# Farama-Foundation/Metaworld

Measured on NVIDIA H100. Metric: env steps/sec MT50 batched (4096 envs/GPU) at 1/2/4/8 H100 vs CPU MuJoCo, higher is better.
Workload: dtype f32

## Files before the change

### include/metaworld_b200.h

```cpp
#ifndef METAWORLD_B200_H
#define METAWORLD_B200_H
#ifdef __cplusplus
extern "C" {
#endif

typedef struct mw_engine mw_engine;

enum mw_status { MW_OK = 0, MW_ERR_CUDA = -1, MW_ERR_ARG = -2, MW_ERR_STATE = -3 };

int mw_sizeof_model(void);
int mw_sizeof_taskconst(void);
int mw_sizeof_envstate(void);
int mw_sizeof_snapshot(void);
const char* mw_last_error(void);
const char* mw_build_info(void);

int mw_create(mw_engine** out, int device, int n_models, const void* models, const void* taskconsts,
              const float* const* meshverts, const int* nmeshvert);
void mw_destroy(mw_engine*);

int mw_set_envs(mw_engine*, int n_envs, const int* env_model);

int mw_build_snapshots(mw_engine*, int n, const int* model_idx, const double* rand_vec ,
                       const double* rand_vec_pass1 , const unsigned char* partially_observable,
// ... 21 lines not shown
int mw_set_options(mw_engine*, int max_episode_steps, int terminate_on_success, unsigned long long seed);
int mw_set_goal_sets(mw_engine*, const int* first , const int* count );

int mw_get_state(mw_engine*, void* out_host);
int mw_set_state(mw_engine*, const void* in_host);
int mw_debug_substeps(mw_engine*, int nstep, const float* ctrl2 , void* stream);
int mw_debug_forward(mw_engine*, const float* ctrl2 , float* dump, void* stream);
int mw_debug_dump_floats(void);
int mw_get_counters(mw_engine*, unsigned long long* out5);

int mw_rebalance(mw_engine*);

int mw_set_profiling(mw_engine*, int on);
int mw_get_env_profile(mw_engine*, unsigned* out );

int mw_get_profile(mw_engine*, unsigned long long* out13);
int mw_get_env_cost(mw_engine*, unsigned* out);

#ifdef __cplusplus
}
#endif
#endif
```

### metaworld_b200/csrc/mw_collide.cuh

```cuda
#pragma once
#include "mw_math.cuh"

#ifndef MW_WARP
#define MW_WARP 32
#endif

enum { G_PLANE = 0, G_HFIELD, G_SPHERE, G_CAPSULE, G_ELLIPSOID, G_CYLINDER, G_BOX, G_MESH };

struct RawCon { creal dist, pos[3], normal[3]; };

struct DShape {
  int type; const creal* pos; const creal* mat; creal size[3]; const float4* vert; int nvert;
};

DEV int plane_sphere_raw(const creal* pn, const creal* pp, const creal* c, creal r, creal margin, RawCon* o) {
  creal t[3]; v3sub(t, c, pp);
  creal dist = v3dot(t, pn) - r;
  if (dist > margin) return 0;
  o->dist = dist; v3copy(o->normal, pn);
  v3addscl(o->pos, c, pn, -(r + (creal)0.5 * dist));
  return 1;
}
DEV int plane_capsule(const DShape& a, const DShape& b, creal margin, RawCon* o) {
  creal n[3], ax[3], c[3]; mat_col(n, a.mat, 2); mat_col(ax, b.mat, 2);
// ... 376 lines not shown
    l[2] = dl[2] >= 0 ? s.size[1] : -s.size[1];
  } else if (s.type == G_CAPSULE) {
    l[0] = l[1] = 0; l[2] = dl[2] >= 0 ? s.size[1] : -s.size[1];
  } else {
    l[0] = l[1] = l[2] = 0;
  }
  mat_mulvec(out, s.mat, l); v3add(out, out, s.pos);
}
DEV creal core_radius(const DShape& s) { return (s.type == G_SPHERE || s.type == G_CAPSULE) ? s.size[0] : (creal)0; }
DEV void support_pair(const DShape& A, const DShape& B, const creal* dir, SV* o, int lane) {
  creal nd[3] = {-dir[0], -dir[1], -dir[2]};
  support_shape(A, dir, o->a, lane);
  support_shape(B, nd, o->b, lane);
  v3sub(o->v, o->a, o->b);
}
DEV void closest_tri(const creal* a, const creal* b, const creal* c, creal* w) {
  creal ab[3], ac[3], ap[3]; v3sub(ab, b, a); v3sub(ac, c, a); v3scl(ap, a, -1);
  creal d1 = v3dot(ab, ap), d2 = v3dot(ac, ap);
  if (d1 <= 0 && d2 <= 0) { w[0] = 1; w[1] = w[2] = 0; return; }
  creal bp[3]; v3scl(bp, b, -1);
  creal d3 = v3dot(ab, bp), d4 = v3dot(ac, bp);
  if (d3 >= 0 && d4 <= d3) { w[1] = 1; w[0] = w[2] = 0; return; }
  creal vc = d1 * d4 - d3 * d2;
  if (vc <= 0 && d1 >= 0 && d3 <= 0) { creal v = d1 / (d1 - d3); w[0] = 1 - v; w[1] = v; w[2] = 0; return; }
  creal cp[3]; v3scl(cp, c, -1);
  creal d5 = v3dot(ab, cp), d6 = v3dot(ac, cp);
  if (d6 >= 0 && d5 <= d6) { w[2] = 1; w[0] = w[1] = 0; return; }
  creal vb = d5 * d2 - d1 * d6;
  if (vb <= 0 && d2 >= 0 && d6 <= 0) { creal x = d2 / (d2 - d6); w[0] = 1 - x; w[1] = 0; w[2] = x; return; }
  creal va = d3 * d6 - d5 * d4;
// ... 207 lines not shown
  } else {
    dist = gr;
    const creal z0 = fmax(-h1, cz - h2), z1 = fmin(h1, cz + h2), zm = (creal)0.5 * (z0 + z1);
    for (int q = 0; q < 3; q++) { n[q] = u[q]; P[q] = A.pos[q] + (r1 + (creal)0.5 * gr) * u[q] + zm * a1[q]; }
  }
  if (dist > margin) return 0;
  o->dist = dist; v3copy(o->normal, n); v3copy(o->pos, P);
  return 1;
}

#define GJK_FINISH() {  \
    creal w4_[3]; simplex_weights(s, n, w4_); v3zero(fwa); v3zero(fwb); \
    for (int i_ = 0; i_ < n && i_ < 3; i_++) { v3addscl(fwa, fwa, s[i_].a, w4_[i_]); v3addscl(fwb, fwb, s[i_].b, w4_[i_]); } \
    creal dv_[3]; v3sub(dv_, fwb, fwa); fdcore = v3norm(dv_); \
    if (fdcore > (creal)1e-10) { outcome = 1; st = ST_DONE; } else { st = ST_G1; k = 0; } }
__device__ __noinline__ int convex_pair(const DShape& A, const DShape& B, creal margin, RawCon* o, EpaSm* E, EpaWs* W, int lane, long long* prof = nullptr) {
  const creal dirs[6][3] = {{1, 0, 0}, {-1, 0, 0}, {0, 1, 0}, {0, -1, 0}, {0, 0, 1}, {0, 0, -1}};
  const creal ra = core_radius(A), rb = core_radius(B);
  enum { ST_GJK0 = 0, ST_GJK, ST_G1, ST_G2, ST_G3, ST_EPA, ST_DONE };
  SV* const s = (SV*)E->fd;
  int n = 0; creal v[3];
  int st = ST_GJK0, git = 0, k = 0, sg = 0;
  int outcome = 0;
  creal ab[3] = {0, 0, 0}, gd[3] = {0, 0, 0}, nn[3] = {0, 0, 0}, vv = 0;
  creal dirl[3] = {1, 0, 0}, fwa[3] = {0, 0, 0}, fwb[3] = {0, 0, 0}, fdcore = 0;
  v3sub(v, A.pos, B.pos);
  if (v3dot(v, v) < (creal)1e-24) { v[0] = 1; v[1] = v[2] = 0; }
  for (int guard = 0; guard < 128; guard++) {
    if (lane == 0) {
      bool query = false;
      while (!query && st != ST_DONE && st != ST_EPA) {
// ... 23 lines not shown
          } else if (n != 3 || sg >= 2) { outcome = 3; st = ST_DONE; }
          else { if (sg == 0) v3copy(dirl, nn); else v3scl(dirl, nn, -1); query = true; }
        }
      }
    }
    const int stb = __shfl_sync(FULLMASK, st, 0);
    if (stb == ST_DONE || stb == ST_EPA) break;
    creal dir[3] = {bcast(dirl[0], 0), bcast(dirl[1], 0), bcast(dirl[2], 0)};
    SV w; support_pair(A, B, dir, &w, lane);
    int need_cs = 0;
    if (lane == 0) {
      if (st == ST_GJK0) { s[0] = w; n = 1; v3copy(v, w.v); st = ST_GJK; git = 0; }
      else if (st == ST_GJK) {
        const creal vw = v3dot(v, w.v);
        if (vv - vw <= (creal)1e-12 * vv || vv - vw <= GJK_TOL * sqrt(vv)) GJK_FINISH()
        else if (vw > 0 && vw / sqrt(vv) - ra - rb > margin + (creal)1e-4) { outcome = 3; st = ST_DONE; }
        else {
          bool dup = false;
          for (int i = 0; i < n; i++) { creal t[3]; v3sub(t, s[i].v, w.v); if (v3dot(t, t) < (creal)1e-24) dup = true; }
          if (dup) GJK_FINISH()
          else { s[n++] = w; need_cs = 1; }
        }
      } else if (st == ST_G1) {
        creal dd[3]; v3sub(dd, w.v, s[0].v);
        if (v3dot(dd, dd) > (creal)1e-20) s[n++] = w;
        k++;
      } else if (st == ST_G2) {
        creal aw[3], cr[3]; v3sub(aw, w.v, s[0].v); v3cross(cr, ab, aw);
        if (v3dot(cr, cr) > (creal)1e-20) s[n++] = w;
        else { sg++; if (sg == 2) { sg = 0; k++; } }
      } else if (st == ST_G3) {
// ... 73 lines not shown
      nf += ne;
      __syncwarp();
    }
  }
  int result = 0;
  RawCon rc; rc.dist = 0; v3zero(rc.pos); v3zero(rc.normal);
  if (lane == 0) {
    creal wa[3] = {0, 0, 0}, wb[3] = {0, 0, 0};
    bool have = false;
    if (outcome == 1) {
      const creal dist = fdcore - ra - rb;
      if (dist <= margin + (creal)1e-4) {
        creal dvec[3]; v3sub(dvec, fwb, fwa);
        v3scl(rc.normal, dvec, 1 / fdcore); rc.dist = dist; have = true;
        v3copy(wa, fwa); v3copy(wb, fwb);
      }
    } else if (outcome == 2 && bestf >= 0) {
      const int i0 = E->fv[0][bestf], i1 = E->fv[1][bestf], i2 = E->fv[2][bestf];
      creal w3[3]; closest_tri(E->vv[i0], E->vv[i1], E->vv[i2], w3);
      const int ids[3] = {i0, i1, i2};
      for (int q = 0; q < 3; q++) for (int c = 0; c < 3; c++) { wa[c] += W->va[ids[q]][c] * w3[q]; wb[c] += W->vb[ids[q]][c] * w3[q]; }
      const creal dist = -E->fd[bestf] - ra - rb;
      if (dist <= margin) { rc.dist = dist; rc.normal[0] = W->fn[0][bestf]; rc.normal[1] = W->fn[1][bestf]; rc.normal[2] = W->fn[2][bestf]; have = true; }
    }
    if (have) {
      for (int q = 0; q < 3; q++) rc.pos[q] = (creal)0.5 * (wa[q] + rc.normal[q] * ra + wb[q] - rc.normal[q] * rb);
      refine_cyl_box(A, B, &rc);
      result = rc.dist <= margin ? 1 : 0;
    }
    if (prof) { prof[10] += eit; prof[11] += git; }
  }
  __syncwarp();
  result = __shfl_sync(FULLMASK, result, 0);
  o->dist = bcast(rc.dist, 0);
  for (int q = 0; q < 3; q++) { o->pos[q] = bcast(rc.pos[q], 0); o->normal[q] = bcast(rc.normal[q], 0); }
  return result;
}
```

### metaworld_b200/csrc/mw_engine.cu

```cuda
#include <cuda_runtime.h>
#include <stdint.h>
#include <stdio.h>
#include <stdlib.h>
#include <string.h>

#include <algorithm>
#include <string>
#include <utility>
#include <vector>

#include "../../include/metaworld_b200.h"
#include "mw_tasks.cuh"

#ifndef WARPS_PER_BLOCK
#define WARPS_PER_BLOCK 7
#endif
#define BLOCK_THREADS (WARPS_PER_BLOCK * 32)
#define MW_ENVPROF_W 20

static thread_local std::string g_err;
static int fail(int code, const std::string& msg) { g_err = msg; return code; }
#define CK(x) do { cudaError_t e_ = (x); if (e_ != cudaSuccess) return fail(MW_ERR_CUDA, std::string(#x ": ") + cudaGetErrorString(e_)); } while (0)

struct EngineDev {
  const unsigned char* models; int model_stride;
  const MwTaskConst* taskconsts;
  const float* const* meshverts;
  MwEnvState* state; MwSnapshot* snaps;
  const int* goal_first; const int* goal_count;
  int* diag;
  EpaWs* epa;
  WarpSpill* spill;
  int slot_by_sm;
  unsigned long long* prof;
  unsigned long long* model_cycles;
  unsigned* env_cost;
  unsigned* env_cycles;
  unsigned* env_prof;
  int n_envs, max_steps, terminate_on_success; unsigned long long seed;
  int autoreset_mode;
};

DEV unsigned mw_smid() { unsigned r; asm volatile("mov.u32 %0, %%smid;" : "=r"(r)); return r; }
DEV size_t scratch_slot(const EngineDev& e, int warp) { return (size_t)(e.slot_by_sm ? mw_smid() : blockIdx.x) * WARPS_PER_BLOCK + warp; }
__global__ void k_nsmid(unsigned* out) { unsigned r; asm volatile("mov.u32 %0, %%nsmid;" : "=r"(r)); *out = r; }

struct BlockShared {
  alignas(16) unsigned char model[(sizeof(MwModel) + 15) / 16 * 16];
  MwTaskConst tc;
  CtaShare cs;
  alignas(8) unsigned long long bar;
};
// ... 11 lines not shown
    asm volatile("fence.proxy.async.shared::cta;" ::: "memory");
  }
  __syncthreads();
  if (threadIdx.x == 0) {
    asm volatile("mbarrier.arrive.expect_tx.shared::cta.b64 _, [%0], %1;" ::"r"(smem_u32(&bs->bar)), "r"(bytes) : "memory");
    asm volatile("cp.async.bulk.shared::cluster.global.mbarrier::complete_tx::bytes [%0], [%1], %2, [%3];" ::"r"(smem_u32(bs->model)), "l"(src), "r"(bytes), "r"(smem_u32(&bs->bar)) : "memory");
  }
  for (int i = threadIdx.x; i < (int)(sizeof(MwTaskConst) / 4); i += blockDim.x) ((int*)&bs->tc)[i] = ((const int*)tc_src)[i];
  unsigned ok = 0;
  do {
    asm volatile("{ .reg .pred p; mbarrier.try_wait.parity.shared::cta.b64 p, [%1], %2; selp.u32 %0, 1, 0, p; }" : "=r"(ok) : "r"(smem_u32(&bs->bar)), "r"(0u) : "memory");
  } while (!ok);
  __syncthreads();
}

DEV void join_cta(BlockShared* bs, WarpShared* wsa, WarpScratch* w, int warp, int live_warps) {
  if (threadIdx.x == 0) { bs->cs.q_head = 0; bs->cs.nwarp = live_warps; bs->cs.peer_stride = (int)sizeof(WarpShared); bs->cs.peer0 = (unsigned char*)wsa; }
  if ((threadIdx.x & 31) == 0) { w->cta = &bs->cs; w->warp_in_cta = warp; w->ncand = 0; w->prof_on = 0; w->nblk1 = mw_tree_split((const MwModel*)bs->model); }
#ifdef MW_CHOL_ONE_CHAIN
  if ((threadIdx.x & 31) == 0) w->nblk1 = ((const MwModel*)bs->model)->nv;
#endif
  __syncwarp();
}
__device__ void eng_forward(const TaskCtx& c, int lane) { mw_forward(c.m, c.meshvert, c.w, lane); }
__device__ void eng_sim(const TaskCtx& c, int nstep, int lane) {
  for (int s = 0; s < nstep; s++) { mw_forward(c.m, c.meshvert, c.w, lane); mw_euler(c.m, c.w, lane); }
}

DEV void load_env(WarpShared* ws, const MwEnvState* src, int lane) {
  ((float4*)&ws->es)[lane] = ((const float4*)src)[lane];
  SYNCW();
  WarpScratch* w = &ws->w;
  if (lane < MW_MAXNQ) { w->qposd[lane] = ws->es.qpos[lane]; w->qpos[lane] = (real)w->qposd[lane]; }
// ... 48 lines not shown
       const int* __restrict__ block_live) {
  extern __shared__ __align__(16) unsigned char smem[];
  BlockShared* bs = (BlockShared*)smem;
  WarpShared* wsa = (WarpShared*)(smem + sizeof(BlockShared));
  const int blk = block_order[blockIdx.x];
  if (block_live && !block_live[blk]) return;
  const int mi = block_model[blk];
  stage_model(bs, e.models + (size_t)mi * e.model_stride, (unsigned)sizeof(bs->model), e.taskconsts + mi);
  const int warp = threadIdx.x >> 5, lane = threadIdx.x & 31;
  if (warp >= block_count[blk]) return;
  const int env = perm[block_start[blk] + warp];
  WarpShared* ws = wsa + warp;
  ws->w.epa = e.epa + scratch_slot(e, warp);
  ws->w.sp = e.spill + scratch_slot(e, warp);
  WarpScratch* w = &ws->w;
  join_cta(bs, wsa, w, warp, block_count[blk]);
  const MwModel* m = (const MwModel*)bs->model;
  load_env(ws, e.state + env, lane);
  const bool ended = DEFERRED && ws->es.ended != 0.f;
  if (lane < 16) w->prof[lane] = 0;
  if (lane == 0) { w->fault = 0; w->prof_on = e.prof != nullptr; }
  SYNCW();
  const long long t_begin = MW_CLK(w);
  const long long t_cta = e.env_cycles ? mw_clock() : 0ll;
  real act[4];
  for (int i = 0; i < 4; i++) act[i] = fmin(fmax((real)actions[4 * env + i], (real)-1), (real)1);
  TaskCtx c; c.m = m; c.tc = &bs->tc; c.w = w; c.s = &ws->es; c.action = act; c.meshvert = e.meshverts[mi];
  if (lane < 3) w->mocap_pos[lane] = fmin(fmax(w->mocap_pos[lane] + act[lane] * (real)0.01, (real)bs->tc.mocap_lo[lane]), (real)bs->tc.mocap_hi[lane]);
  if (lane == 0) { w->ctrl[0] = (real)actions[4 * env + 3]; w->ctrl[1] = -(real)actions[4 * env + 3]; }
  SYNCW();
  int iters = 0, dropped = 0, ncon_max = 0, nefc_max = 0, solver_work = 0, cand_total = 0;
// ... 26 lines not shown
    ws->info[7] = (term || trunc) ? 1.f : 0.f;
    if (!ended) {
      reward[env] = (float)rew; terminated[env] = term; truncated[env] = trunc;
      if (info_stride >= 9) { info_out[(size_t)env * info_stride + 7] = (float)rew; info_out[(size_t)env * info_stride + 8] = (float)((int)term + 2 * (int)trunc); }
      { bool fin = isfinite((float)rew); for (int i = 0; i < 39; i++) fin = fin && isfinite(ws->obs[i]); if (!fin) w->fault |= MW_FAULT_NONFINITE; }
      e.diag[3 * env] += dropped; e.diag[3 * env + 1] += iters; e.diag[3 * env + 2] |= w->fault;
    } else if (e.autoreset_mode == MW_AUTORESET_DISABLED) e.diag[3 * env + 2] |= MW_FAULT_STEP_AFTER_END;
    w->prof[7] = MW_CLK(w) - t_phys; w->prof[8] = MW_CLK(w) - t_begin;
    const long long own = w->prof[8] - w->prof[12];
    e.env_cost[env] = (unsigned)solver_work;
    if (e.env_cycles) { long long d = mw_clock() - t_cta; e.env_cycles[env] = (unsigned)(d > 0xFFFFFFFFll ? 0xFFFFFFFFll : d); }
    w->prof[6] = own - w->prof[7] - (w->prof[0] + w->prof[1] + w->prof[3] + w->prof[4] + w->prof[5]);
  }
  SYNCW();
  if (e.prof) {
    if (lane < 13) atomicAdd(e.prof + lane, (unsigned long long)w->prof[lane]);
    if (lane == 0 && e.model_cycles) { atomicAdd(e.model_cycles + 2 * mi, (unsigned long long)w->prof[8]); atomicAdd(e.model_cycles + 2 * mi + 1, 1ull); }
    if (e.env_prof) {
      if (lane < 13) e.env_prof[MW_ENVPROF_W * env + lane] = (unsigned)(w->prof[lane] > 0xFFFFFFFFll ? 0xFFFFFFFFll : w->prof[lane]);
      if (lane == 13) e.env_prof[MW_ENVPROF_W * env + 13] = (unsigned)iters;
      if (lane == 14) e.env_prof[MW_ENVPROF_W * env + 14] = (unsigned)ncon_max;
      if (lane == 15) e.env_prof[MW_ENVPROF_W * env + 15] = (unsigned)nefc_max;
      if (lane == 16) e.env_prof[MW_ENVPROF_W * env + 16] = (unsigned)blockIdx.x;
      if (lane == 17) e.env_prof[MW_ENVPROF_W * env + 17] = (unsigned)cand_total;
    }
  }
  done = ws->info[7] != 0.f;
  if (ended) {
    if (e.autoreset_mode == MW_AUTORESET_DISABLED) return;
    if (lane < INFO_N) info_out[(size_t)env * info_stride + lane] = 0.f;
    if (lane == 0) {
      reward[env] = 0.f; terminated[env] = 0; truncated[env] = 0;
      if (info_stride >= 9) { info_out[(size_t)env * info_stride + 7] = 0.f; info_out[(size_t)env * info_stride + 8] = 0.f; }
    }
  } else {
    if (lane < INFO_N) info_out[(size_t)env * info_stride + lane] = ws->info[lane];
    if (!done || DEFERRED) {
      if (DEFERRED && done) {
        if (final_info && lane == 7) final_info[(size_t)env * 8 + 7] = ws->es.ep_return;
// ... 251 lines not shown
    }
    keys[i] = key;
  }
  bitonic_sort_u64(keys, P);
  for (int i = threadIdx.x; i < n_blocks; i += blockDim.x) block_order[i] = (int)(keys[i] & 0xFFFFFFFFull);
}

struct mw_engine {
  int device = 0, n_models = 0, n_envs = 0, model_stride = 0;
  unsigned char* d_models = nullptr; MwTaskConst* d_tc = nullptr; float** d_meshptrs = nullptr;
  std::vector<float*> meshbufs;
  MwEnvState* d_state = nullptr; MwSnapshot* d_snaps = nullptr; int snap_cap = 0, n_snaps = 0;
  int *d_goal_first = nullptr, *d_goal_count = nullptr, *d_diag = nullptr;
  EpaWs* d_epa = nullptr; WarpSpill* d_spill = nullptr; size_t epa_cap = 0; int slot_by_sm = 0, nsmid = 0;
  unsigned long long* d_prof = nullptr; unsigned long long* d_model_cycles = nullptr; unsigned* d_env_prof = nullptr; int profiling = 0;
  unsigned* d_env_cost = nullptr; unsigned* d_env_cycles = nullptr; int order_by_cycles = 1, head_warps = 0; int *d_block_order = nullptr, *d_model_first = nullptr, *d_model_count = nullptr; int n_sorted_models = 0;
  std::vector<int> h_faults;
  std::vector<int> env_model; std::vector<int> model_order;
  int n_blocks = 0; int *d_block_model = nullptr, *d_block_start = nullptr, *d_block_count = nullptr, *d_perm = nullptr;
  int n_blocks_total = 0, n_split = 0, split_warps = 4, n_sm = 0; float split_frac = 0.f;
  int *d_split_head = nullptr, *d_split_alt = nullptr, *d_split_state = nullptr, *d_block_live = nullptr;
  int max_steps = 500, terminate_on_success = 0; unsigned long long seed = 0; int autoreset_mode = MW_AUTORESET_SAME_STEP;
  unsigned long long launches = 0, env_steps = 0;
  EngineDev dev() const {
    EngineDev e; e.models = d_models; e.model_stride = model_stride; e.taskconsts = d_tc; e.meshverts = d_meshptrs;
    e.state = d_state; e.snaps = d_snaps; e.goal_first = d_goal_first; e.goal_count = d_goal_count; e.diag = d_diag; e.epa = d_epa; e.spill = d_spill; e.slot_by_sm = slot_by_sm; e.prof = profiling ? d_prof : nullptr; e.model_cycles = d_model_cycles; e.env_cost = d_env_cost; e.env_cycles = order_by_cycles ? d_env_cycles : nullptr; e.env_prof = profiling ? d_env_prof : nullptr;
    e.n_envs = n_envs; e.max_steps = max_steps; e.terminate_on_success = terminate_on_success; e.seed = seed; e.autoreset_mode = autoreset_mode; return e;
  }
};

static void make_blocks(int n_models, const std::vector<int>& item_model, std::vector<int>& bm, std::vector<int>& bstart, std::vector<int>& bcount, std::vector<int>& perm,
                        const std::vector<int>* order = nullptr, int head = 0) {
  bm.clear(); bstart.clear(); bcount.clear(); perm.clear();
  for (int oi = 0; oi < n_models; oi++) {
    const int mi = order && (int)order->size() == n_models ? (*order)[oi] : oi;
    int first = (int)perm.size();
    for (int i = 0; i < (int)item_model.size(); i++) if (item_model[i] == mi) perm.push_back(i);
    int cnt = (int)perm.size() - first;
    int h = head < 0 ? cnt % WARPS_PER_BLOCK : head;
    if (h <= 0 || h > WARPS_PER_BLOCK) h = WARPS_PER_BLOCK;
    for (int o = 0; o < cnt; ) {
// ... 119 lines not shown
  CK(cudaFuncSetAttribute(k_evaluate, cudaFuncAttributeMaxDynamicSharedMemorySize, (int)smem_bytes()));
  { const char* k = getenv("MW_B200_ORDER_KEY"); if (k && !strcmp(k, "work")) E->order_by_cycles = 0; }
  { const char* k = getenv("MW_B200_HEAD_WARPS"); if (k) E->head_warps = atoi(k); }
  { const char* k = getenv("MW_B200_SPLIT_FRAC"); if (k) E->split_frac = (float)atof(k); }
  { const char* k = getenv("MW_B200_SPLIT_WARPS"); if (k) E->split_warps = atoi(k); }
  { cudaDeviceProp pr; CK(cudaGetDeviceProperties(&pr, device)); E->n_sm = pr.multiProcessorCount; }
  *out = E;
  return MW_OK;
}

void mw_destroy(mw_engine* E) {
  if (!E) return;
  cudaSetDevice(E->device);
  cudaFree(E->d_models); cudaFree(E->d_tc); cudaFree(E->d_meshptrs);
  for (float* p : E->meshbufs) cudaFree(p);
  cudaFree(E->d_state); cudaFree(E->d_snaps); cudaFree(E->d_goal_first); cudaFree(E->d_goal_count); cudaFree(E->d_diag); cudaFree(E->d_epa); cudaFree(E->d_spill); cudaFree(E->d_prof); cudaFree(E->d_model_cycles); cudaFree(E->d_env_prof); cudaFree(E->d_env_cost); cudaFree(E->d_env_cycles); cudaFree(E->d_block_order); cudaFree(E->d_model_first); cudaFree(E->d_model_count);
  cudaFree(E->d_block_model); cudaFree(E->d_block_start); cudaFree(E->d_block_count); cudaFree(E->d_perm);
  cudaFree(E->d_split_head); cudaFree(E->d_split_alt); cudaFree(E->d_split_state); cudaFree(E->d_block_live);
  delete E;
}

int mw_set_envs(mw_engine* E, int n_envs, const int* env_model) {
  if (!E || n_envs <= 0 || !env_model) return fail(MW_ERR_ARG, "mw_set_envs: bad arguments");
  CK(cudaSetDevice(E->device));
  std::vector<int> im(env_model, env_model + n_envs), bm, bs, bc, perm;
  for (int v : im) if (v < 0 || v >= E->n_models) return fail(MW_ERR_ARG, "mw_set_envs: model index out of range");
  E->env_model = im;
  E->n_envs = n_envs;
  E->h_faults.assign(n_envs, 0);
  if (upload_env_blocks(E)) return MW_ERR_CUDA;
  if (E->d_env_cost) cudaFree(E->d_env_cost);
  CK(cudaMalloc((void**)&E->d_env_cost, sizeof(unsigned) * n_envs));
  CK(cudaMemset(E->d_env_cost, 0, sizeof(unsigned) * n_envs));
  if (E->d_env_cycles) cudaFree(E->d_env_cycles);
  CK(cudaMalloc((void**)&E->d_env_cycles, sizeof(unsigned) * n_envs));
  CK(cudaMemset(E->d_env_cycles, 0, sizeof(unsigned) * n_envs));
  if (E->d_state) cudaFree(E->d_state);
  CK(cudaMalloc((void**)&E->d_state, sizeof(MwEnvState) * n_envs));
  CK(cudaMemset(E->d_state, 0, sizeof(MwEnvState) * n_envs));
  if (E->d_env_prof) { cudaFree(E->d_env_prof); E->d_env_prof = nullptr; }
  if (E->profiling) { CK(cudaMalloc((void**)&E->d_env_prof, sizeof(unsigned) * MW_ENVPROF_W * n_envs)); CK(cudaMemset(E->d_env_prof, 0, sizeof(unsigned) * MW_ENVPROF_W * n_envs)); }
  if (E->d_diag) cudaFree(E->d_diag);
  CK(cudaMalloc((void**)&E->d_diag, sizeof(int) * 3 * n_envs));
  CK(cudaMemset(E->d_diag, 0, sizeof(int) * 3 * n_envs));
  return MW_OK;
}

int mw_build_snapshots(mw_engine* E, int n, const int* model_idx, const double* rand_vec, const double* rand_vec_pass1, const unsigned char* partial, int* ids_out) {
  if (!E || n <= 0 || !model_idx || !rand_vec || !partial) return fail(MW_ERR_ARG, "mw_build_snapshots: bad arguments");
  CK(cudaSetDevice(E->device));
  if (E->n_snaps + n > E->snap_cap) {
// ... 196 lines not shown
}
int mw_get_env_profile(mw_engine* E, unsigned* out) {
  if (!E || !out || !E->d_env_prof) return fail(MW_ERR_STATE, "mw_get_env_profile: profiling is off (mw_set_profiling)");
  CK(cudaSetDevice(E->device));
  CK(cudaMemcpy(out, E->d_env_prof, sizeof(unsigned) * MW_ENVPROF_W * E->n_envs, cudaMemcpyDeviceToHost));
  return MW_OK;
}

int mw_get_env_cost(mw_engine* E, unsigned* out) {
  if (!E || !out || !E->d_env_cost) return fail(MW_ERR_ARG, "mw_get_env_cost");
  CK(cudaSetDevice(E->device));
  CK(cudaMemcpy(out, E->d_env_cost, sizeof(unsigned) * E->n_envs, cudaMemcpyDeviceToHost));
  return MW_OK;
}

int mw_get_profile(mw_engine* E, unsigned long long* out13) {
  if (!E || !out13) return fail(MW_ERR_ARG, "mw_get_profile");
  CK(cudaSetDevice(E->device));
  CK(cudaMemcpy(out13, E->d_prof, sizeof(unsigned long long) * 13, cudaMemcpyDeviceToHost));
  CK(cudaMemset(E->d_prof, 0, sizeof(unsigned long long) * 16));
  return MW_OK;
}

}
```

### metaworld_b200/csrc/mw_model.h

```cpp
#pragma once
#define MW_MAXLINK 12
#define MW_MAXDOF 17
#define MW_MAXNQ 18
#define MW_MAXGEOM 40
#define MW_MAXPAIR 384
#define MW_MAXPARAM 32
#define MW_MAXFRAME 32
#define MW_NPARAM 12
struct MwModel {
  double qpos0d[18];
  int nlink;
  int nq;
  int nv;
  int ngeom;
  int npair;
  int nframe;
  int nmeshvert;
  int pad0;
  float timestep;
  float solver_scale;
  float gravity[3];
  float tolerance;
  float impratio;
  float pad1;
// ... 37 lines not shown
  int geom_type[40];
  int geom_link[40];
  int geom_shift[40];
  int geom_meshadr[40];
  int geom_meshnum[40];
  int geom_srcid[40];
  float geom_pos[40][3];
  float geom_mat[40][9];
  float geom_size[40][3];
  float geom_rbound[40];
  float geom_invw[40][2];
  float geom_aabb[40][6];
  unsigned char pair_g1[384];
  unsigned char pair_g2[384];
  unsigned char pair_param[384];
  float param[32][12];
  int frame_link[32];
  int frame_shift[32];
  float frame_pos[32][3];
  float frame_quat[32][4];
};
static_assert(sizeof(MwModel) == 11128, "MwModel layout mismatch with lower.py");
#define F_HAND 0
#define F_RCLAW 1
#define F_LCLAW 2
#define F_RPAD 3
#define F_LPAD 4
#define F_REE 5
#define F_LEE 6
#define F_TASK0 7
```

### metaworld_b200/csrc/mw_physics.cuh

```cuda
#pragma once
#include "mw_model.h"
#include "mw_collide.cuh"

#define NVP 17
#ifndef MW_SMCON
#define MW_SMCON 48
#endif
#ifndef MW_MAXCON
#define MW_MAXCON 80
#endif
#define MW_MAXSCALAR 24
#define MW_SMEFC (MW_MAXSCALAR + 4 * MW_SMCON)
#define MW_MAXEFC (MW_MAXSCALAR + 4 * MW_MAXCON)

enum { JT_FREE = 0, JT_BALL, JT_SLIDE, JT_HINGE };

struct ConvRes { RawCon r; int hit, pad; };

struct Contact {
  real pos[3], frame[9], dist, mu, fr1, fr3;
  real H[10];
  real fn;
  short row, prm;
  unsigned char dim, g1, g2, hzone;
// ... 9 lines not shown
struct WarpSpill;

struct WarpScratch {
  real lpos[MW_MAXLINK][3], lquat[MW_MAXLINK][4], lmat[MW_MAXLINK][9];
  real lcom[MW_MAXLINK][3], lIw[MW_MAXLINK][9];
  real daxis[MW_MAXDOF][3], danchor[MW_MAXDOF][3];
  real qpos[MW_MAXNQ], qvel[MW_MAXDOF], warm[MW_MAXDOF];
  double qposd[MW_MAXNQ], lposd[MW_MAXLINK][3], lquatd[MW_MAXLINK][4];
  real ctrl[2], mocap_pos[3], mocap_quat[4], shift[3];
  real qfrc_smooth[MW_MAXDOF], qacc_smooth[MW_MAXDOF], qfrc_con[MW_MAXDOF], qacc[MW_MAXDOF];
  real vMa[MW_MAXDOF], vSearch[MW_MAXDOF], vMs[MW_MAXDOF], vTmp[MW_MAXDOF];
  real M[MW_MAXDOF * NVP], H[MW_MAXDOF * NVP];
  alignas(16) real U[MW_UWORDS];
  EpaWs* epa;
  WarpSpill* sp;
  real eD[MW_SMEFC], eAref[MW_SMEFC], eJar[MW_SMEFC], eJv[MW_SMEFC], eF[MW_SMEFC], eHd[MW_MAXSCALAR];
  Contact con[MW_SMCON];
  unsigned short cand[MW_MAXCAND];
  unsigned char achunk[MW_MAXCON];
  CtaShare* cta; int warp_in_cta, ncand;
  int nblk1;
  int ncon, nefc, nscalar, nweld, solver_iter, ncon_dropped;
  int fault;
  int prof_on;
  long long prof[16];
};

struct WarpSpill {
  real J[(MW_MAXEFC - MW_SMEFC) * NVP];
  real eD[MW_MAXEFC - MW_SMEFC], eAref[MW_MAXEFC - MW_SMEFC], eJar[MW_MAXEFC - MW_SMEFC], eJv[MW_MAXEFC - MW_SMEFC], eF[MW_MAXEFC - MW_SMEFC];
// ... 428 lines not shown
      while (k >= cs->q_cnt[o]) { k -= cs->q_cnt[o]; o++; }
      WarpScratch* ow = (WarpScratch*)(cs->peer0 + (size_t)o * cs->peer_stride);
      const creal* ogpose = (const creal*)ow->U;
      ConvRes* ores = (ConvRes*)((unsigned char*)ogpose + MW_MAXGEOM * 12 * sizeof(creal) + sizeof(EpaSm));
      const int pp = ow->cand[k];
      int h1 = m->pair_g1[pp], h2 = m->pair_g2[pp];
      DShape a, b; mw_load_shape(m, ogpose, meshvert, h1, &a); mw_load_shape(m, ogpose, meshvert, h2, &b);
      creal mg = m->param[m->pair_param[pp]][0];
      RawCon r1; int c1;
      if (a.type == G_PLANE) {
        creal n[3], nd[3], sp[3], t[3]; mat_col(n, a.mat, 2); v3scl(nd, n, -1);
        support_shape(b, nd, sp, lane);
        v3sub(t, sp, a.pos);
        r1.dist = v3dot(t, n); v3copy(r1.normal, n); v3addscl(r1.pos, sp, n, -(creal)0.5 * r1.dist);
        c1 = r1.dist <= mg;
      } else { long long tc = MW_CLK(w); c1 = convex_pair(a, b, mg, &r1, esm, epa, lane, w->prof); if (lane == 0) { w->prof[2] += MW_CLK(w) - tc; w->prof[9] += 1; } }
      if (lane == 0) { ores[k].hit = c1; if (c1) ores[k].r = r1; }
    }
  }
  __syncthreads();
  {
    int nhit = 0;
    for (int k = 0; k < ncand; k++) nhit += cres[k].hit != 0;
    const int nA = ncon < MW_MAXCON ? ncon : MW_MAXCON;
    int j = nA + nhit - 1, ai = nA - 1, hk = ncand - 1;
    SYNCW();
    while (nhit > 0 && j >= 0) {
      while (hk >= 0 && !cres[hk].hit) hk--;
      const bool take_hit = hk >= 0 && (ai < 0 || (int)w->achunk[ai] <= (int)(w->cand[hk] >> 5));
      if (take_hit) {
        if (j < MW_MAXCON && lane == 0) mw_store_contact(m, w, j, cres[hk].r, w->cand[hk]);
// ... 495 lines not shown
```

### metaworld_b200/engine.py

```python
from __future__ import annotations

import ctypes as C
import os

import numpy as np

from . import lower, modelzoo
from .tasks import TASKS, TaskSpec

_LIB = None
_LIB64 = None
_HERE = os.path.dirname(os.path.abspath(__file__))
SO_PATH = os.environ.get("MW_B200_LIB") or os.path.join(_HERE, "libmwb200.so")
SO64_PATH = os.path.join(_HERE, "libmwb200_f64.so")

TASKCONST_DTYPE = np.dtype([("task_id", "i4"), ("nframe_task", "i4"), ("main_geom", "i4"), ("pad", "i4"),
                            ("hand_init", "f4", 3), ("mocap_lo", "f4", 3), ("mocap_hi", "f4", 3),
                            ("goal_lo", "f4", 3), ("goal_hi", "f4", 3), ("movable_pos0", "f4", 3), ("p", "f4", 16)])
ENVSTATE_DTYPE = np.dtype([("qpos", "f8", 18), ("qvel", "f4", 17), ("warm", "f4", 17), ("mocap_pos", "f4", 3),
                           ("prev_obs", "f4", 18), ("shift", "f4", 3), ("target", "f4", 3), ("obj_init", "f4", 3),
                           ("init_tcp", "f4", 3), ("scal", "f4", 16), ("path_len", "f4"),
                           ("partially_observable", "f4"), ("snapshot", "f4"), ("episode", "f4"), ("ep_return", "f4"),
                           ("ended", "f4"), ("pad", "f4", 3)])
SNAPSHOT_DTYPE = np.dtype([("st", ENVSTATE_DTYPE), ("obs", "f4", 39), ("pad", "f4", 25)])
# ... 247 lines not shown

    def debug_substeps(self, nstep, ctrl=(0.0, 0.0)):
        c = np.array(ctrl, dtype=np.float32)
        _ck(lib().mw_debug_substeps(self.h, int(nstep), c.ctypes.data, self._stream()))

    def debug_forward(self, ctrl=(0.0, 0.0)):
        nf = lib().mw_debug_dump_floats()
        buf = self.torch.zeros(self.n_envs, nf, device=self.device)
        c = np.array(ctrl, dtype=np.float32)
        _ck(lib().mw_debug_forward(self.h, c.ctypes.data, self._p(buf), self._stream()))
        a = buf.cpu().numpy()
        ncw = (nf - 17 - 4)
        return a[:, :ncw].reshape(self.n_envs, -1, 12), a[:, ncw:ncw + 17], a[:, ncw + 17:]

    PROFILE_KEYS = ["kin_mass", "collide", "gjk_epa", "constraints", "bias_smooth", "solver", "euler_glue", "obs_reward", "step",
                    "n_convex_pairs", "n_epa_expansions", "n_gjk_iters", "barrier_wait"]

    def profile(self):
        out = np.zeros(13, dtype=np.uint64)
        self.torch.cuda.synchronize(self.device)
        _ck(lib().mw_get_profile(self.h, out.ctypes.data))
        return dict(zip(self.PROFILE_KEYS, (int(x) for x in out)))

    def set_profiling(self, on=True):
        _ck(lib().mw_set_profiling(self.h, int(bool(on))))

    def env_profile(self):
        out = np.zeros((self.n_envs, 20), dtype=np.uint32)
        self.torch.cuda.synchronize(self.device)
        _ck(lib().mw_get_env_profile(self.h, out.ctypes.data))
        return out

    def env_cost(self):
        out = np.zeros(self.n_envs, dtype=np.uint32)
# ... 14 lines not shown
```

### metaworld_b200/lower.py

```python
from __future__ import annotations

import numpy as np

from . import mjcf
from .mjcf import (GEOM_MESH, GEOM_PLANE, JNT_FREE, JNT_HINGE, JNT_SLIDE, quat2mat, quat_conj, quat_mul, quat_norm)

MAXLINK, MAXDOF, MAXNQ, MAXGEOM, MAXPAIR, MAXPARAM, MAXFRAME = 12, 17, 18, 40, 384, 32, 32
NPARAM = 12

FIELDS = [
    ("qpos0d", "f8", (MAXNQ,)),
    ("nlink", "i4", ()), ("nq", "i4", ()), ("nv", "i4", ()), ("ngeom", "i4", ()), ("npair", "i4", ()),
    ("nframe", "i4", ()), ("nmeshvert", "i4", ()), ("pad0", "i4", ()),
    ("timestep", "f4", ()), ("solver_scale", "f4", ()), ("gravity", "f4", (3,)), ("tolerance", "f4", ()),
    ("impratio", "f4", ()), ("pad1", "f4", ()),
    ("link_parent", "i4", (MAXLINK,)), ("link_jtype", "i4", (MAXLINK,)), ("link_qadr", "i4", (MAXLINK,)),
    ("link_dadr", "i4", (MAXLINK,)), ("link_shift", "i4", (MAXLINK,)), ("link_dofmask", "u4", (MAXLINK,)),
    ("link_pos", "f4", (MAXLINK, 3)), ("link_quat", "f4", (MAXLINK, 4)), ("link_jaxis", "f4", (MAXLINK, 3)),
    ("link_jpos", "f4", (MAXLINK, 3)), ("link_mass", "f4", (MAXLINK,)), ("link_com", "f4", (MAXLINK, 3)),
    ("link_inertia", "f4", (MAXLINK, 6)),
    ("dof_link", "i4", (MAXDOF,)), ("dof_qadr", "i4", (MAXDOF,)), ("dof_limited", "i4", (MAXDOF,)),
    ("dof_damping", "f4", (MAXDOF,)), ("dof_armature", "f4", (MAXDOF,)), ("dof_invweight", "f4", (MAXDOF,)),
    ("dof_lo", "f4", (MAXDOF,)), ("dof_hi", "f4", (MAXDOF,)), ("dof_stiffness", "f4", (MAXDOF,)),
    ("dof_springref", "f4", (MAXDOF,)), ("qpos0", "f4", (MAXNQ,)),
    ("act_dof", "i4", (2,)), ("act_kp", "f4", (2,)), ("act_lo", "f4", (2,)), ("act_hi", "f4", (2,)),
    ("weld_link", "i4", ()), ("weld_pos", "f4", (3,)), ("weld_quat", "f4", (4,)), ("weld_invw", "f4", (2,)),
    ("weld_solref", "f4", (2,)), ("weld_solimp", "f4", (5,)), ("weld_torquescale", "f4", ()),
    ("mocap_pos0", "f4", (3,)), ("mocap_quat0", "f4", (4,)),
    ("geom_type", "i4", (MAXGEOM,)), ("geom_link", "i4", (MAXGEOM,)), ("geom_shift", "i4", (MAXGEOM,)),
    ("geom_meshadr", "i4", (MAXGEOM,)), ("geom_meshnum", "i4", (MAXGEOM,)), ("geom_srcid", "i4", (MAXGEOM,)),
    ("geom_pos", "f4", (MAXGEOM, 3)), ("geom_mat", "f4", (MAXGEOM, 9)), ("geom_size", "f4", (MAXGEOM, 3)),
    ("geom_rbound", "f4", (MAXGEOM,)), ("geom_invw", "f4", (MAXGEOM, 2)),
    ("geom_aabb", "f4", (MAXGEOM, 6)),
    ("pair_g1", "u1", (MAXPAIR,)), ("pair_g2", "u1", (MAXPAIR,)), ("pair_param", "u1", (MAXPAIR,)),
    ("param", "f4", (MAXPARAM, NPARAM)),
    ("frame_link", "i4", (MAXFRAME,)), ("frame_shift", "i4", (MAXFRAME,)), ("frame_pos", "f4", (MAXFRAME, 3)),
    ("frame_quat", "f4", (MAXFRAME, 4)),
]

DTYPE = np.dtype([(n, t, s) for n, t, s in FIELDS], align=True)

ROBOT_FRAMES = [("body", "hand"), ("body", "rightclaw"), ("body", "leftclaw"), ("body", "rightpad"),
                ("body", "leftpad"), ("site", "rightEndEffector"), ("site", "leftEndEffector")]
F_HAND, F_RCLAW, F_LCLAW, F_RPAD, F_LPAD, F_REE, F_LEE, F_TASK0 = range(8)


def emit_header() -> str:
    ctype = {"i4": "int", "u4": "unsigned int", "f4": "float", "u1": "unsigned char", "f8": "double"}
    lines = ["/* GENERATED by metaworld_b200/lower.py:emit_header -- do not edit. */", "#pragma once",
             f"#define MW_MAXLINK {MAXLINK}", f"#define MW_MAXDOF {MAXDOF}", f"#define MW_MAXNQ {MAXNQ}",
             f"#define MW_MAXGEOM {MAXGEOM}", f"#define MW_MAXPAIR {MAXPAIR}", f"#define MW_MAXPARAM {MAXPARAM}",
             f"#define MW_MAXFRAME {MAXFRAME}", f"#define MW_NPARAM {NPARAM}", "struct MwModel {"]
    for n, t, s in FIELDS:
        dims = "".join(f"[{d}]" for d in s)
        lines.append(f"  {ctype[t]} {n}{dims};")
    lines.append("};")
    lines.append(f"static_assert(sizeof(MwModel) == {DTYPE.itemsize}, \"MwModel layout mismatch with lower.py\");")
    for i, nm in enumerate(["F_HAND", "F_RCLAW", "F_LCLAW", "F_RPAD", "F_LPAD", "F_REE", "F_LEE", "F_TASK0"]):
        lines.append(f"#define {nm} {i}")
    return "\n".join(lines) + "\n"


class Lowered:
    def __init__(self):
        self.rec = np.zeros((), dtype=DTYPE)
        self.meshvert = np.zeros((0, 3), dtype=np.float32)
        self.frame_names = []
# ... 201 lines not shown
        r["geom_meshnum"][i] = 0
        if a["geom_type"][g] == GEOM_MESH:
            mid = int(a["geom_dataid"][g])
            if mid not in mesh_adr:
                mesh_adr[mid] = sum(len(x) for x in mv)
                mv.append(np.asarray(m.meshes[mid]["vert"], dtype=np.float32))
            r["geom_meshadr"][i] = mesh_adr[mid]
            r["geom_meshnum"][i] = len(m.meshes[mid]["vert"])
        out.geom_names.append(m.names["geom"][g])
        out.geom_src.append(g)
    r["ngeom"] = len(used)
    out.meshvert = np.concatenate(mv, axis=0) if mv else np.zeros((0, 3), dtype=np.float32)
    r["nmeshvert"] = len(out.meshvert)

    params = []
    for k, (g1, g2) in enumerate(pairs):
        prm = mix_params(a, g1, g2)
        key = tuple(np.round(prm, 12))
        if key not in params:
            params.append(key)
        r["pair_g1"][k], r["pair_g2"][k], r["pair_param"][k] = cid[g1], cid[g2], params.index(key)
    assert len(params) <= MAXPARAM, len(params)
    for i, p in enumerate(params):
        r["param"][i] = p
    r["npair"] = len(pairs)

    frames = list(ROBOT_FRAMES) + list(task_frames)
    assert len(frames) <= MAXFRAME
    for i, (kind, name) in enumerate(frames):
        if kind == "body":
            b = m.names["body"].index(name)
            fp, fq = rel_pos[b], rel_quat[b]
        elif kind == "geom":
            g = m.names["geom"].index(name)
            b = a["geom_bodyid"][g]
            fp, fq = _compose(rel_pos[b], rel_quat[b], a["geom_pos"][g], a["geom_quat"][g])
        elif kind == "site":
            s = m.names["site"].index(name)
            b = a["site_bodyid"][s]
            fp, fq = _compose(rel_pos[b], rel_quat[b], a["site_pos"][s], a["site_quat"][s])
        else:
            raise ValueError(kind)
        l = link_of_body[b]
        r["frame_link"][i] = l
        r["frame_shift"][i] = int(l < 0 and shifted[b])
        r["frame_pos"][i] = fp
        r["frame_quat"][i] = fq
        out.frame_names.append((kind, name))
    r["nframe"] = len(frames)
    return out


def mix_params(a, g1, g2):
    assert a["geom_priority"][g1] == a["geom_priority"][g2]
    margin = max(a["geom_margin"][g1], a["geom_margin"][g2])
    gap = max(a["geom_gap"][g1], a["geom_gap"][g2])
    dim = max(a["geom_condim"][g1], a["geom_condim"][g2])
    s1, s2 = a["geom_solmix"][g1], a["geom_solmix"][g2]
    mix = s1 / (s1 + s2)
    r1, r2 = a["geom_solref"][g1], a["geom_solref"][g2]
    if r1[0] > 0 and r2[0] > 0:
        solref = mix * r1 + (1 - mix) * r2
    else:
        solref = np.minimum(r1, r2)
    solimp = mix * a["geom_solimp"][g1] + (1 - mix) * a["geom_solimp"][g2]
    fr = np.maximum(a["geom_friction"][g1], a["geom_friction"][g2])
    assert dim in (1, 3, 4)
# ... 2 lines not shown
```

Before: 1.331 million.

## Cache per-pair separating axes across steps to skip GJK for separated convex pairs

Adds a per-env, per-convex-pair float4 hint buffer that stores the last separating direction (or contact normal). Before running full GJK/EPA, a single support-pair query along the cached axis checks whether the shapes are still separated beyond the margin, and skips convex_pair if so. This targets repeated GJK iterations on pairs that stay apart between steps. In exchange it adds global memory traffic per pair, grows the model struct by a cslot table, and adds profiling counters.

```diff
diff --git a/include/metaworld_b200.h b/include/metaworld_b200.h
--- a/include/metaworld_b200.h
+++ b/include/metaworld_b200.h
@@ -59,7 +59,7 @@
 int mw_set_profiling(mw_engine*, int on);
 int mw_get_env_profile(mw_engine*, unsigned* out );
 
-int mw_get_profile(mw_engine*, unsigned long long* out13);
+int mw_get_profile(mw_engine*, unsigned long long* out15);
 int mw_get_env_cost(mw_engine*, unsigned* out);
 
 #ifdef __cplusplus
diff --git a/metaworld_b200/csrc/mw_collide.cuh b/metaworld_b200/csrc/mw_collide.cuh
--- a/metaworld_b200/csrc/mw_collide.cuh
+++ b/metaworld_b200/csrc/mw_collide.cuh
@@ -414,6 +414,19 @@
   support_shape(B, nd, o->b, lane);
   v3sub(o->v, o->a, o->b);
 }
+#define SEP_APART 1.f
+#define SEP_HIT 2.f
+DEV int sep_hint_test(const DShape& A, const DShape& B, creal margin, const float4* hint, int lane) {
+  const float4 h = *hint;
+  if (h.w != SEP_APART) return -1;
+  creal n[3] = {h.x, h.y, h.z};
+  const creal nn = v3dot(n, n);
+  if (!(nn > (creal)1e-30 && nn < (creal)1e30)) return -1;
+  v3scl(n, n, 1 / sqrt(nn));
+  SV w; support_pair(A, B, n, &w, lane);
+  return -v3dot(n, w.v) - core_radius(A) - core_radius(B) > margin + (creal)1e-4 ? 1 : 0;
+}
+DEV void sep_hint_store(float4* hint, const creal* n, float flag) { *hint = float4{(float)n[0], (float)n[1], (float)n[2], flag}; }
 DEV void closest_tri(const creal* a, const creal* b, const creal* c, creal* w) {
   creal ab[3], ac[3], ap[3]; v3sub(ab, b, a); v3sub(ac, c, a); v3scl(ap, a, -1);
   creal d1 = v3dot(ab, ap), d2 = v3dot(ac, ap);
@@ -651,7 +664,8 @@
     for (int i_ = 0; i_ < n && i_ < 3; i_++) { v3addscl(fwa, fwa, s[i_].a, w4_[i_]); v3addscl(fwb, fwb, s[i_].b, w4_[i_]); } \
     creal dv_[3]; v3sub(dv_, fwb, fwa); fdcore = v3norm(dv_); \
     if (fdcore > (creal)1e-10) { outcome = 1; st = ST_DONE; } else { st = ST_G1; k = 0; } }
-__device__ __noinline__ int convex_pair(const DShape& A, const DShape& B, creal margin, RawCon* o, EpaSm* E, EpaWs* W, int lane, long long* prof = nullptr) {
+__device__ __noinline__ int convex_pair(const DShape& A, const DShape& B, creal margin, RawCon* o, EpaSm* E, EpaWs* W, int lane, long long* prof = nullptr,
+                                        float4* hint = nullptr) {
   const creal dirs[6][3] = {{1, 0, 0}, {-1, 0, 0}, {0, 1, 0}, {0, -1, 0}, {0, 0, 1}, {0, 0, -1}};
   const creal ra = core_radius(A), rb = core_radius(B);
   enum { ST_GJK0 = 0, ST_GJK, ST_G1, ST_G2, ST_G3, ST_EPA, ST_DONE };
@@ -705,7 +719,10 @@
       else if (st == ST_GJK) {
         const creal vw = v3dot(v, w.v);
         if (vv - vw <= (creal)1e-12 * vv || vv - vw <= GJK_TOL * sqrt(vv)) GJK_FINISH()
-        else if (vw > 0 && vw / sqrt(vv) - ra - rb > margin + (creal)1e-4) { outcome = 3; st = ST_DONE; }
+        else if (vw > 0 && vw / sqrt(vv) - ra - rb > margin + (creal)1e-4) {
+          outcome = 3; st = ST_DONE;
+          if (hint) sep_hint_store(hint, dirl, SEP_APART);
+        }
         else {
           bool dup = false;
           for (int i = 0; i < n; i++) { creal t[3]; v3sub(t, s[i].v, w.v); if (v3dot(t, t) < (creal)1e-24) dup = true; }
@@ -809,7 +826,7 @@
         creal dvec[3]; v3sub(dvec, fwb, fwa);
         v3scl(rc.normal, dvec, 1 / fdcore); rc.dist = dist; have = true;
         v3copy(wa, fwa); v3copy(wb, fwb);
-      }
+      } else if (hint) { creal dvec[3]; v3sub(dvec, fwb, fwa); sep_hint_store(hint, dvec, SEP_APART); }
     } else if (outcome == 2 && bestf >= 0) {
       const int i0 = E->fv[0][bestf], i1 = E->fv[1][bestf], i2 = E->fv[2][bestf];
       creal w3[3]; closest_tri(E->vv[i0], E->vv[i1], E->vv[i2], w3);
@@ -822,6 +839,7 @@
       for (int q = 0; q < 3; q++) rc.pos[q] = (creal)0.5 * (wa[q] + rc.normal[q] * ra + wb[q] - rc.normal[q] * rb);
       refine_cyl_box(A, B, &rc);
       result = rc.dist <= margin ? 1 : 0;
+      if (hint && result) sep_hint_store(hint, rc.normal, SEP_HIT);
     }
     if (prof) { prof[10] += eit; prof[11] += git; }
   }
diff --git a/metaworld_b200/csrc/mw_engine.cu b/metaworld_b200/csrc/mw_engine.cu
--- a/metaworld_b200/csrc/mw_engine.cu
+++ b/metaworld_b200/csrc/mw_engine.cu
@@ -36,6 +36,7 @@
   unsigned long long* model_cycles;
   unsigned* env_cost;
   unsigned* env_cycles;
+  float4* sep_hint;
   unsigned* env_prof;
   int n_envs, max_steps, terminate_on_success; unsigned long long seed;
   int autoreset_mode;
@@ -77,9 +78,9 @@
   __syncthreads();
 }
 
-DEV void join_cta(BlockShared* bs, WarpShared* wsa, WarpScratch* w, int warp, int live_warps) {
+DEV void join_cta(BlockShared* bs, WarpShared* wsa, WarpScratch* w, int warp, int live_warps, float4* sep = nullptr) {
   if (threadIdx.x == 0) { bs->cs.q_head = 0; bs->cs.nwarp = live_warps; bs->cs.peer_stride = (int)sizeof(WarpShared); bs->cs.peer0 = (unsigned char*)wsa; }
-  if ((threadIdx.x & 31) == 0) { w->cta = &bs->cs; w->warp_in_cta = warp; w->ncand = 0; w->prof_on = 0; w->nblk1 = mw_tree_split((const MwModel*)bs->model); }
+  if ((threadIdx.x & 31) == 0) { w->cta = &bs->cs; w->warp_in_cta = warp; w->ncand = 0; w->prof_on = 0; w->nblk1 = mw_tree_split((const MwModel*)bs->model); w->sep = sep; }
 #ifdef MW_CHOL_ONE_CHAIN
   if ((threadIdx.x & 31) == 0) w->nblk1 = ((const MwModel*)bs->model)->nv;
 #endif
@@ -158,7 +159,7 @@
   ws->w.epa = e.epa + scratch_slot(e, warp);
   ws->w.sp = e.spill + scratch_slot(e, warp);
   WarpScratch* w = &ws->w;
-  join_cta(bs, wsa, w, warp, block_count[blk]);
+  join_cta(bs, wsa, w, warp, block_count[blk], e.sep_hint + (size_t)env * MW_NCONV);
   const MwModel* m = (const MwModel*)bs->model;
   load_env(ws, e.state + env, lane);
   const bool ended = DEFERRED && ws->es.ended != 0.f;
@@ -215,7 +216,7 @@
   }
   SYNCW();
   if (e.prof) {
-    if (lane < 13) atomicAdd(e.prof + lane, (unsigned long long)w->prof[lane]);
+    if (lane < 15) atomicAdd(e.prof + lane, (unsigned long long)w->prof[lane]);
     if (lane == 0 && e.model_cycles) { atomicAdd(e.model_cycles + 2 * mi, (unsigned long long)w->prof[8]); atomicAdd(e.model_cycles + 2 * mi + 1, 1ull); }
     if (e.env_prof) {
       if (lane < 13) e.env_prof[MW_ENVPROF_W * env + lane] = (unsigned)(w->prof[lane] > 0xFFFFFFFFll ? 0xFFFFFFFFll : w->prof[lane]);
@@ -224,6 +225,7 @@
       if (lane == 15) e.env_prof[MW_ENVPROF_W * env + 15] = (unsigned)nefc_max;
       if (lane == 16) e.env_prof[MW_ENVPROF_W * env + 16] = (unsigned)blockIdx.x;
       if (lane == 17) e.env_prof[MW_ENVPROF_W * env + 17] = (unsigned)cand_total;
+      if (lane == 18 || lane == 19) e.env_prof[MW_ENVPROF_W * env + lane] = (unsigned)w->prof[lane - 5];
     }
   }
   done = ws->info[7] != 0.f;
@@ -505,6 +507,7 @@
   int *d_goal_first = nullptr, *d_goal_count = nullptr, *d_diag = nullptr;
   EpaWs* d_epa = nullptr; WarpSpill* d_spill = nullptr; size_t epa_cap = 0; int slot_by_sm = 0, nsmid = 0;
   unsigned long long* d_prof = nullptr; unsigned long long* d_model_cycles = nullptr; unsigned* d_env_prof = nullptr; int profiling = 0;
+  float4* d_sep_hint = nullptr;
   unsigned* d_env_cost = nullptr; unsigned* d_env_cycles = nullptr; int order_by_cycles = 1, head_warps = 0; int *d_block_order = nullptr, *d_model_first = nullptr, *d_model_count = nullptr; int n_sorted_models = 0;
   std::vector<int> h_faults;
   std::vector<int> env_model; std::vector<int> model_order;
@@ -516,6 +519,7 @@
   EngineDev dev() const {
     EngineDev e; e.models = d_models; e.model_stride = model_stride; e.taskconsts = d_tc; e.meshverts = d_meshptrs;
     e.state = d_state; e.snaps = d_snaps; e.goal_first = d_goal_first; e.goal_count = d_goal_count; e.diag = d_diag; e.epa = d_epa; e.spill = d_spill; e.slot_by_sm = slot_by_sm; e.prof = profiling ? d_prof : nullptr; e.model_cycles = d_model_cycles; e.env_cost = d_env_cost; e.env_cycles = order_by_cycles ? d_env_cycles : nullptr; e.env_prof = profiling ? d_env_prof : nullptr;
+    e.sep_hint = d_sep_hint;
     e.n_envs = n_envs; e.max_steps = max_steps; e.terminate_on_success = terminate_on_success; e.seed = seed; e.autoreset_mode = autoreset_mode; return e;
   }
 };
@@ -665,7 +669,7 @@
   cudaSetDevice(E->device);
   cudaFree(E->d_models); cudaFree(E->d_tc); cudaFree(E->d_meshptrs);
   for (float* p : E->meshbufs) cudaFree(p);
-  cudaFree(E->d_state); cudaFree(E->d_snaps); cudaFree(E->d_goal_first); cudaFree(E->d_goal_count); cudaFree(E->d_diag); cudaFree(E->d_epa); cudaFree(E->d_spill); cudaFree(E->d_prof); cudaFree(E->d_model_cycles); cudaFree(E->d_env_prof); cudaFree(E->d_env_cost); cudaFree(E->d_env_cycles); cudaFree(E->d_block_order); cudaFree(E->d_model_first); cudaFree(E->d_model_count);
+  cudaFree(E->d_state); cudaFree(E->d_snaps); cudaFree(E->d_goal_first); cudaFree(E->d_goal_count); cudaFree(E->d_diag); cudaFree(E->d_epa); cudaFree(E->d_spill); cudaFree(E->d_prof); cudaFree(E->d_model_cycles); cudaFree(E->d_env_prof); cudaFree(E->d_env_cost); cudaFree(E->d_env_cycles); cudaFree(E->d_sep_hint); cudaFree(E->d_block_order); cudaFree(E->d_model_first); cudaFree(E->d_model_count);
   cudaFree(E->d_block_model); cudaFree(E->d_block_start); cudaFree(E->d_block_count); cudaFree(E->d_perm);
   cudaFree(E->d_split_head); cudaFree(E->d_split_alt); cudaFree(E->d_split_state); cudaFree(E->d_block_live);
   delete E;
@@ -686,6 +690,9 @@
   if (E->d_env_cycles) cudaFree(E->d_env_cycles);
   CK(cudaMalloc((void**)&E->d_env_cycles, sizeof(unsigned) * n_envs));
   CK(cudaMemset(E->d_env_cycles, 0, sizeof(unsigned) * n_envs));
+  if (E->d_sep_hint) cudaFree(E->d_sep_hint);
+  CK(cudaMalloc((void**)&E->d_sep_hint, sizeof(float4) * MW_NCONV * n_envs));
+  CK(cudaMemset(E->d_sep_hint, 0, sizeof(float4) * MW_NCONV * n_envs));
   if (E->d_state) cudaFree(E->d_state);
   CK(cudaMalloc((void**)&E->d_state, sizeof(MwEnvState) * n_envs));
   CK(cudaMemset(E->d_state, 0, sizeof(MwEnvState) * n_envs));
@@ -912,10 +919,10 @@
   return MW_OK;
 }
 
-int mw_get_profile(mw_engine* E, unsigned long long* out13) {
-  if (!E || !out13) return fail(MW_ERR_ARG, "mw_get_profile");
-  CK(cudaSetDevice(E->device));
-  CK(cudaMemcpy(out13, E->d_prof, sizeof(unsigned long long) * 13, cudaMemcpyDeviceToHost));
+int mw_get_profile(mw_engine* E, unsigned long long* out15) {
+  if (!E || !out15) return fail(MW_ERR_ARG, "mw_get_profile");
+  CK(cudaSetDevice(E->device));
+  CK(cudaMemcpy(out15, E->d_prof, sizeof(unsigned long long) * 15, cudaMemcpyDeviceToHost));
   CK(cudaMemset(E->d_prof, 0, sizeof(unsigned long long) * 16));
   return MW_OK;
 }
diff --git a/metaworld_b200/csrc/mw_model.h b/metaworld_b200/csrc/mw_model.h
--- a/metaworld_b200/csrc/mw_model.h
+++ b/metaworld_b200/csrc/mw_model.h
@@ -7,6 +7,7 @@
 #define MW_MAXPARAM 32
 #define MW_MAXFRAME 32
 #define MW_NPARAM 12
+#define MW_NCONV 128
 struct MwModel {
   double qpos0d[18];
   int nlink;
@@ -75,13 +76,14 @@
   unsigned char pair_g1[384];
   unsigned char pair_g2[384];
   unsigned char pair_param[384];
+  unsigned char pair_cslot[384];
   float param[32][12];
   int frame_link[32];
   int frame_shift[32];
   float frame_pos[32][3];
   float frame_quat[32][4];
 };
-static_assert(sizeof(MwModel) == 11128, "MwModel layout mismatch with lower.py");
+static_assert(sizeof(MwModel) == 11512, "MwModel layout mismatch with lower.py");
 #define F_HAND 0
 #define F_RCLAW 1
 #define F_LCLAW 2
diff --git a/metaworld_b200/csrc/mw_physics.cuh b/metaworld_b200/csrc/mw_physics.cuh
--- a/metaworld_b200/csrc/mw_physics.cuh
+++ b/metaworld_b200/csrc/mw_physics.cuh
@@ -47,6 +47,7 @@
   alignas(16) real U[MW_UWORDS];
   EpaWs* epa;
   WarpSpill* sp;
+  float4* sep;
   real eD[MW_SMEFC], eAref[MW_SMEFC], eJar[MW_SMEFC], eJv[MW_SMEFC], eF[MW_SMEFC], eHd[MW_MAXSCALAR];
   Contact con[MW_SMCON];
   unsigned short cand[MW_MAXCAND];
@@ -505,7 +506,19 @@
         v3sub(t, sp, a.pos);
         r1.dist = v3dot(t, n); v3copy(r1.normal, n); v3addscl(r1.pos, sp, n, -(creal)0.5 * r1.dist);
         c1 = r1.dist <= mg;
-      } else { long long tc = MW_CLK(w); c1 = convex_pair(a, b, mg, &r1, esm, epa, lane, w->prof); if (lane == 0) { w->prof[2] += MW_CLK(w) - tc; w->prof[9] += 1; } }
+      } else {
+        const long long tc = MW_CLK(w);
+        float4* hint = nullptr;
+#ifndef MW_NO_SEPCACHE
+        if (ow->sep && m->pair_cslot[pp] < MW_NCONV) hint = ow->sep + m->pair_cslot[pp];
+#endif
+        const int ht = hint ? sep_hint_test(a, b, mg, hint, lane) : -1;
+        c1 = ht == 1 ? 0 : convex_pair(a, b, mg, &r1, esm, epa, lane, w->prof, hint);
+        if (lane == 0) {
+          w->prof[2] += MW_CLK(w) - tc; w->prof[9] += 1;
+          if (w->prof_on) { w->prof[13] += ht >= 0; w->prof[14] += ht == 1; }
+        }
+      }
       if (lane == 0) { ores[k].hit = c1; if (c1) ores[k].r = r1; }
     }
   }
diff --git a/metaworld_b200/engine.py b/metaworld_b200/engine.py
--- a/metaworld_b200/engine.py
+++ b/metaworld_b200/engine.py
@@ -285,10 +285,10 @@
         return a[:, :ncw].reshape(self.n_envs, -1, 12), a[:, ncw:ncw + 17], a[:, ncw + 17:]
 
     PROFILE_KEYS = ["kin_mass", "collide", "gjk_epa", "constraints", "bias_smooth", "solver", "euler_glue", "obs_reward", "step",
-                    "n_convex_pairs", "n_epa_expansions", "n_gjk_iters", "barrier_wait"]
+                    "n_convex_pairs", "n_epa_expansions", "n_gjk_iters", "barrier_wait", "n_sep_tested", "n_sep_rejected"]
 
     def profile(self):
-        out = np.zeros(13, dtype=np.uint64)
+        out = np.zeros(len(self.PROFILE_KEYS), dtype=np.uint64)
         self.torch.cuda.synchronize(self.device)
         _ck(lib().mw_get_profile(self.h, out.ctypes.data))
         return dict(zip(self.PROFILE_KEYS, (int(x) for x in out)))
diff --git a/metaworld_b200/lower.py b/metaworld_b200/lower.py
--- a/metaworld_b200/lower.py
+++ b/metaworld_b200/lower.py
@@ -3,10 +3,13 @@
 import numpy as np
 
 from . import mjcf
-from .mjcf import (GEOM_MESH, GEOM_PLANE, JNT_FREE, JNT_HINGE, JNT_SLIDE, quat2mat, quat_conj, quat_mul, quat_norm)
+from .mjcf import (GEOM_BOX, GEOM_CAPSULE, GEOM_MESH, GEOM_PLANE, GEOM_SPHERE, JNT_FREE, JNT_HINGE, JNT_SLIDE, quat2mat,
+                   quat_conj, quat_mul, quat_norm)
 
 MAXLINK, MAXDOF, MAXNQ, MAXGEOM, MAXPAIR, MAXPARAM, MAXFRAME = 12, 17, 18, 40, 384, 32, 32
 NPARAM = 12
+MAXCONV = 128
+NO_CSLOT = 255
 
 FIELDS = [
     ("qpos0d", "f8", (MAXNQ,)),
@@ -33,6 +36,7 @@
     ("geom_rbound", "f4", (MAXGEOM,)), ("geom_invw", "f4", (MAXGEOM, 2)),
     ("geom_aabb", "f4", (MAXGEOM, 6)),
     ("pair_g1", "u1", (MAXPAIR,)), ("pair_g2", "u1", (MAXPAIR,)), ("pair_param", "u1", (MAXPAIR,)),
+    ("pair_cslot", "u1", (MAXPAIR,)),
     ("param", "f4", (MAXPARAM, NPARAM)),
     ("frame_link", "i4", (MAXFRAME,)), ("frame_shift", "i4", (MAXFRAME,)), ("frame_pos", "f4", (MAXFRAME, 3)),
     ("frame_quat", "f4", (MAXFRAME, 4)),
@@ -50,7 +54,8 @@
     lines = ["/* GENERATED by metaworld_b200/lower.py:emit_header -- do not edit. */", "#pragma once",
              f"#define MW_MAXLINK {MAXLINK}", f"#define MW_MAXDOF {MAXDOF}", f"#define MW_MAXNQ {MAXNQ}",
              f"#define MW_MAXGEOM {MAXGEOM}", f"#define MW_MAXPAIR {MAXPAIR}", f"#define MW_MAXPARAM {MAXPARAM}",
-             f"#define MW_MAXFRAME {MAXFRAME}", f"#define MW_NPARAM {NPARAM}", "struct MwModel {"]
+             f"#define MW_MAXFRAME {MAXFRAME}", f"#define MW_NPARAM {NPARAM}", f"#define MW_NCONV {MAXCONV}",
+             "struct MwModel {"]
     for n, t, s in FIELDS:
         dims = "".join(f"[{d}]" for d in s)
         lines.append(f"  {ctype[t]} {n}{dims};")
@@ -282,13 +287,19 @@
     r["nmeshvert"] = len(out.meshvert)
 
     params = []
+    nconv = 0
     for k, (g1, g2) in enumerate(pairs):
         prm = mix_params(a, g1, g2)
         key = tuple(np.round(prm, 12))
         if key not in params:
             params.append(key)
         r["pair_g1"][k], r["pair_g2"][k], r["pair_param"][k] = cid[g1], cid[g2], params.index(key)
+        r["pair_cslot"][k] = NO_CSLOT
+        if general_convex(a["geom_type"][g1], a["geom_type"][g2]):
+            r["pair_cslot"][k] = nconv
+            nconv += 1
     assert len(params) <= MAXPARAM, len(params)
+    assert nconv <= MAXCONV, nconv
     for i, p in enumerate(params):
         r["param"][i] = p
     r["npair"] = len(pairs)
@@ -319,6 +330,11 @@
     return out
 
 
+def general_convex(t1, t2) -> bool:
+    analytic3 = (GEOM_SPHERE, GEOM_CAPSULE, GEOM_BOX)
+    return t1 != GEOM_PLANE and not (t1 in analytic3 and t2 in analytic3)
+
+
 def mix_params(a, g1, g2):
     assert a["geom_priority"][g1] == a["geom_priority"][g2]
     margin = max(a["geom_margin"][g1], a["geom_margin"][g2])
```

After: 1.372 million (median of 6 runs). 3.1% higher.
